# henry123-boy/Level-S2FM_official

Hardware: AMD Instinct MI355X
Metric: rendered rays/sec (fwd+bwd) (higher is better)
Workload: dtype f32; 1 GPU; C2: ETH3D bounds, 1024 rays x 128 samples per GPU, dual field, L16/F2/T19 hash grid, fwd+loss+bwd; rays_per_gpu=1024, samples_per_ray=128, dual_field=True, parallelism=dp1 (rays sharded by view)

## Files before the change

level-s2fm_official_amd/csrc/bin_items.h:

```cpp
#pragma once

#include "render_common.h"

namespace {

constexpr int kAccSlots = 2 << kSlabShift;
constexpr int kSlabBins = 128 << (13 - kSlabShift);
constexpr int kBins = kSlabBins;
#ifndef LS2FM_FILL_TILE
#define LS2FM_FILL_TILE 256
#endif
constexpr int kCountThreads = LS2FM_FILL_TILE;
constexpr int kFillThreads = LS2FM_FILL_TILE;
constexpr int kFillCap = kFillThreads * 17 / 4;
#ifndef LS2FM_FILL_WIN
#define LS2FM_FILL_WIN (LS2FM_FILL_TILE * 17 / 8)
#endif
constexpr int kFillWin = LS2FM_FILL_WIN;
#ifndef LS2FM_ACC_THREADS
#define LS2FM_ACC_THREADS 1024
#endif
constexpr int kAccThreads = LS2FM_ACC_THREADS;
#ifndef LS2FM_ACC_BATCH
#define LS2FM_ACC_BATCH 4
// ... 184 lines not shown

inline int* scan_ticket(const BinMeta& bm) { return reinterpret_cast<int*>(bm.level_bound) + 48; }
__device__ __forceinline__ int* scan_ticket_dev(const BinMeta& bm) { return reinterpret_cast<int*>(bm.level_bound) + 48; }
__host__ __device__ __forceinline__ int* acc_claim(const BinMeta& bm) { return reinterpret_cast<int*>(bm.level_bound) + 50; }

__device__ __forceinline__ int wave_scan_incl_i32(int v, int lane) {
#pragma unroll
    for (int o = 1; o < 64; o <<= 1) {
        const int t = __shfl_up(v, o, 64);
        if (lane >= o) v += t;
    }
    return v;
}

constexpr int kScanTiles = 512;
constexpr int kScanArenaInts = kScanTiles * kScanGroup + (512 / kScanGroup) * kScanGroup + LS2FM_MAX_LEVELS + 1;
[[maybe_unused]] __device__ void scan_job_run(const ScanJob& sj, const int job, const int tid, const int nt, int* arena) {
    int* stage = arena;
    int (*chunk_sum)[kScanGroup] = reinterpret_cast<int (*)[kScanGroup]>(arena + kScanTiles * kScanGroup);
    int* level_total = arena + kScanTiles * kScanGroup + (512 / kScanGroup) * kScanGroup;
    int& s_last = level_total[LS2FM_MAX_LEVELS];
    const BinMeta& bm = sj.bm;
    const int l = job / kScanJobsPerLevel;
    const int sub = tid % kScanGroup, ch = tid / kScanGroup, n_ch = nt / kScanGroup;
    const int b0 = (job % kScanJobsPerLevel) * kScanGroup;
    int* blk = bm.tile + (int64_t)l * bm.n_tiles * kBins + b0;
    int carry = 0;
    for (int base = 0; base < bm.n_tiles; base += kScanTiles) {
        const int nt_here = bm.n_tiles - base < kScanTiles ? bm.n_tiles - base : kScanTiles;
        for (int e = tid; e < nt_here * kScanGroup; e += nt)
            stage[e] = blk[(int64_t)(base + e / kScanGroup) * kBins + e % kScanGroup];
        __syncthreads();
        const int per = (nt_here + n_ch - 1) / n_ch;
        const int t0 = ch * per, t1 = t0 + per < nt_here ? t0 + per : nt_here;
        int sum = 0;
        for (int t = t0; t < t1; ++t) sum += stage[t * kScanGroup + sub];
        chunk_sum[ch][sub] = sum;
        __syncthreads();
        int run = carry, total = carry;
        for (int q = 0; q < n_ch; ++q) {
            const int v = chunk_sum[q][sub];
            if (q < ch) run += v;
            total += v;
        }
// ... 4 lines not shown
        }
        carry = total;
        __syncthreads();
        for (int e = tid; e < nt_here * kScanGroup; e += nt)
            blk[(int64_t)(base + e / kScanGroup) * kBins + e % kScanGroup] = stage[e];
        __syncthreads();
    }
    if (ch == 0) __hip_atomic_store(&bm.count[l * kBins + b0 + sub], carry, __ATOMIC_RELAXED, __HIP_MEMORY_SCOPE_AGENT);
    asm volatile("s_waitcnt vmcnt(0)" ::: "memory");
    __syncthreads();
    if (tid == 0) s_last = atomicAdd(scan_ticket_dev(bm), 1) == sj.n_levels * kScanJobsPerLevel - 1;
    __syncthreads();
    if (!s_last) return;
    const int lane = tid & 63, wave = tid >> 6, n_waves = nt >> 6;
    constexpr int kChunks = (kBins + 63) / 64;
    constexpr int kHeld = 4;
    int held[kHeld][kChunks];
#pragma unroll
    for (int h = 0; h < kHeld; ++h) {
        const int lv = wave + h * n_waves;
        int tot = 0;
#pragma unroll
        for (int c = 0; c < kChunks; ++c) {
            const int bb = 64 * c + lane;
            held[h][c] = (lv < sj.n_levels && bb < kBins)
                             ? __hip_atomic_load(&bm.count[lv * kBins + bb], __ATOMIC_RELAXED, __HIP_MEMORY_SCOPE_AGENT) : 0;
            tot += held[h][c];
        }
#pragma unroll
        for (int o = 32; o > 0; o >>= 1) tot += __shfl_xor(tot, o, 64);
        if (lane == 0 && lv < LS2FM_MAX_LEVELS) level_total[lv] = tot;
    }
    __syncthreads();
#pragma unroll
    for (int h = 0; h < kHeld; ++h) {
        const int lv = wave + h * n_waves;
        if (lv >= sj.n_levels) continue;
        int before = 0;
        for (int q = 0; q < lv; ++q) before += level_total[q];
        int run2 = 0;
#pragma unroll
        for (int c = 0; c < kChunks; ++c) {
            const int bb = 64 * c + lane;
            const int cnt = held[h][c];
            const int incl = wave_scan_incl_i32(cnt, lane);
            if (bb < kBins) bm.start[lv * kBins + bb] = before + run2 + incl - cnt;
            run2 += __shfl(incl, 63, 64);
        }
    }
    if (tid == 0) *scan_ticket_dev(bm) = 0;
}

struct ZeroJob { float4* a; int64_t na; float4* b; int64_t nb; float4* c; int64_t nc; int blocks; };
__device__ __forceinline__ void zero_job_run(const ZeroJob& z, const int job, const int tid, const int nt) {
    const float4 zero = make_float4(0.f, 0.f, 0.f, 0.f);
    const int64_t stride = (int64_t)z.blocks * nt;
    for (int64_t i = (int64_t)job * nt + tid; i < z.na; i += stride) z.a[i] = zero;
    for (int64_t i = (int64_t)job * nt + tid; i < z.nb; i += stride) z.b[i] = zero;
    for (int64_t i = (int64_t)job * nt + tid; i < z.nc; i += stride) z.c[i] = zero;
// ... 4 lines not shown
```

level-s2fm_official_amd/csrc/loss_head.hip:

```cpp
#include "bin_items.h"

namespace {

constexpr int kLossThreads = 256;
constexpr int kLossMaxBlocks = 512;
constexpr int kSums = 8;

struct LossIn {
    const float* rgb; const float* rgb_gt;
    const float* normals;
    const float* depth; const float* depth_ref;
    const uint8_t* mask_eik; const uint8_t* mask_dc; const uint8_t* mask_mse;
    int64_t n_rays; int32_t n_samples;
};

__device__ __forceinline__ float smooth_l1(float d) { const float a = fabsf(d); return a < 1.0f ? 0.5f * d * d : a - 0.5f; }
__device__ __forceinline__ float smooth_l1_grad(float d) { return fabsf(d) < 1.0f ? d : (d > 0.f ? 1.0f : -1.0f); }
__device__ __forceinline__ float sign_of(float d) { return d > 0.f ? 1.0f : (d < 0.f ? -1.0f : 0.f); }

__device__ __forceinline__ void finish_terms(const double* s, const float* w, float* terms, double* sums_out) {
    const float rgb = (float)(s[0] / s[1]);
    const float eik = (float)(s[2] / s[3]);
    const float dc = s[5] > 0.0 ? (float)(s[4] / s[5]) : 0.f;
    const float mse = (float)(s[6] / s[7]);
    terms[0] = rgb; terms[1] = eik; terms[2] = dc; terms[3] = mse;
    terms[4] = fmaf(w[2], dc, fmaf(w[1], eik, w[0] * rgb));
    terms[5] = terms[4];
    terms[6] = -10.0f * log10f(mse);
    terms[7] = 0.f;
    for (int k = 0; k < kSums; ++k) sums_out[k] = s[k];
}

__global__ void __launch_bounds__(kLossThreads)
loss_head_fwd_kernel(LossIn in, const float* __restrict__ weights, double* __restrict__ partial, unsigned* __restrict__ ticket,
                     double* __restrict__ sums_out, float* __restrict__ terms) {
    __shared__ double red[kLossThreads / 64][kSums];
    __shared__ bool last;
    const int tid = threadIdx.x, lane = tid & 63, wave = tid >> 6;
    const int64_t n_points = in.n_rays * in.n_samples;
    const int64_t stride = (int64_t)gridDim.x * kLossThreads;
    double s[kSums];
#pragma unroll
    for (int k = 0; k < kSums; ++k) s[k] = 0.0;
    for (int64_t i = (int64_t)blockIdx.x * kLossThreads + tid; i < n_points; i += stride) {
        const int64_t r = i / in.n_samples;
        if (in.mask_eik && !in.mask_eik[r]) continue;
// ... 83 lines not shown
            const float d = in.rgb[3 * i + c] - in.rgb_gt[3 * i + c];
            float v = g_rgb * sign_of(d);
            if (m) v = fmaf(g_mse * 2.0f, d, v);
            d_rgb[3 * i + c] = v;
        }
        float gd = 0.f;
        if (in.depth_ref && (!in.mask_dc || in.mask_dc[i])) gd = g_dc * smooth_l1_grad(in.depth_ref[i] - in.depth[i]);
        d_depth[i] = -gd;
        if (d_depth_ref) d_depth_ref[i] = gd;
    }
}

constexpr int kPostThreads = 512;
__global__ void __launch_bounds__(kPostThreads)
post_shade_kernel(ls2fm_loss_spec loss, const float* __restrict__ lpart, int64_t n_rays, int64_t r_pad, int n_samples, ScanJob scan) {
    __shared__ int arena[kScanArenaInts];
    const int tid = threadIdx.x, lane = tid & 63, wave = tid >> 6;
    if (blockIdx.x > 0) {
        scan_job_run(scan, (int)blockIdx.x - 1, tid, kPostThreads, arena);
        return;
    }
    if (loss.rgb_gt == nullptr) return;
    double (*red)[kSums] = reinterpret_cast<double (*)[kSums]>(arena);
    static_assert(sizeof(double) * (kPostThreads / 64) * kSums <= sizeof(int) * kScanArenaInts, "reduction buffer fits");
    double s[kSums];
#pragma unroll
    for (int k = 0; k < kSums; ++k) s[k] = 0.0;
    for (int64_t r = tid; r < n_rays; r += kPostThreads) {
        s[0] += (double)lpart[0 * r_pad + r];
        s[1] += 3.0;
        if (ls2fm_in_eik(loss, r)) { s[2] += (double)lpart[1 * r_pad + r]; s[3] += (double)n_samples; }
        if (loss.depth_ref != nullptr && (loss.mask_dc == nullptr || loss.mask_dc[r])) {
            s[4] += (double)ls2fm_smooth_l1(loss.depth_ref[r] - lpart[2 * r_pad + r]);
            s[5] += 1.0;
        }
        if (ls2fm_in_mse(loss, r)) { s[6] += (double)lpart[3 * r_pad + r]; s[7] += 3.0; }
    }
#pragma unroll
    for (int k = 0; k < kSums; ++k) {
        double v = s[k];
#pragma unroll
        for (int o = 32; o > 0; o >>= 1) v += __shfl_xor(v, o, 64);
        if (lane == 0) red[wave][k] = v;
    }
    __syncthreads();
    if (tid < kSums) {
        double v = 0.0;
        for (int q = 0; q < kPostThreads / 64; ++q) v += red[q][tid];
        if ((tid & 1) && loss.count_scale > 1u) v *= (double)loss.count_scale;
        red[0][tid] = v;
    }
    __syncthreads();
    if (tid == 0) finish_terms(red[0], loss.weights, loss.terms, loss.sums);
}

__global__ void terms_from_sums_kernel(const double* __restrict__ sums, const float* __restrict__ weights, float* __restrict__ terms) {
    double s[kSums], keep[kSums];
    for (int k = 0; k < kSums; ++k) s[k] = sums[k];
    finish_terms(s, weights, terms, keep);
}

}

int ls2fm_launch_post_shade(const ls2fm_loss_spec* loss, const float* ray_part, int64_t n_rays, int n_samples,
                            const ls2fm_grid_desc* scan_grid, int64_t n_points, float* bins_ws, hipStream_t stream) {
    if (!loss && !scan_grid) return LS2FM_OK;
    ls2fm_loss_spec ls{};
    if (loss) ls = *loss;
// ... 64 lines not shown
```

level-s2fm_official_amd/csrc/render_common.h:

```cpp
#pragma once

#include "ls2fm_device.h"

enum ls2fm_prof_id {
    LS2FM_PROF_PREP = 0, LS2FM_PROF_ENCODE_SDF, LS2FM_PROF_ENCODE_RAD, LS2FM_PROF_SHADE_FWD, LS2FM_PROF_SHADE_BWD,
    LS2FM_PROF_WGRAD_GEO, LS2FM_PROF_WGRAD_TAIL, LS2FM_PROF_SCATTER_SDF, LS2FM_PROF_SCATTER_RAD, LS2FM_PROF_FINALIZE,
    LS2FM_PROF_SDF_EVAL, LS2FM_PROF_SPHERE_TRACE, LS2FM_PROF_BIN, LS2FM_PROF_LOSS_FWD,
    LS2FM_PROF_LOSS_BWD, LS2FM_PROF_WGRAD_MLP, LS2FM_PROF_POSE, LS2FM_PROF_ENCODE_PAIR, LS2FM_PROF_COUNT
};
bool ls2fm_prof_enabled();
void ls2fm_prof_begin(int id, hipStream_t stream);
void ls2fm_prof_end(int id, hipStream_t stream);

struct SideCtx { hipStream_t side; hipEvent_t fork, mid, join; };
bool ls2fm_side_stream(SideCtx* out, hipStream_t caller);
int ls2fm_join_on_error(bool forked, const SideCtx& sc, hipStream_t caller, int status);
int* ls2fm_async_error_word(hipStream_t stream);
int ls2fm_device_cus();

constexpr int kHidden = LS2FM_HIDDEN;
constexpr int kOut = LS2FM_FEAT + 1;
constexpr int kInMax = 3 + 2 * LS2FM_MAX_LEVELS;
constexpr int kView = LS2FM_VIEW_ENC;
constexpr int kRadIn = 3 + 3 + kView + 2 * LS2FM_FEAT;
// ... 147 lines not shown
    return (q & 1) ? cosf(x) : sinf(x);
}

static inline bool same_grid_geometry(const ls2fm_grid_desc* a, const ls2fm_grid_desc* b) {
    if (a->n_levels != b->n_levels) return false;
    for (int l = 0; l < a->n_levels; ++l)
        if (a->scale[l] != b->scale[l] || a->resolution[l] != b->resolution[l] || a->size[l] != b->size[l] ||
            a->hashed[l] != b->hashed[l])
            return false;
    return true;
}

int64_t ls2fm_bins_workspace_floats(int n_levels, int64_t n_points);
int ls2fm_explicit_levels(const ls2fm_grid_desc* grid, int dual, int n_samples);

struct WsLayout {
    int64_t p, p_pad, r_pad;
    int l1, l2, dual;
    int64_t packed, e1, j1, e2, sdfv, nrm, rgbs, fe, fe2, rout, lpart;
    int64_t rec1, rec2, rpt, bins, v, p3, gf, dz, gf2, dzr, renc, dexyz, dlen, mpart, wg, dbeta, smax;
    int64_t total;
};

#ifndef LS2FM_SLAB_SHIFT
#define LS2FM_SLAB_SHIFT 13
#endif
constexpr int kSlabShift = LS2FM_SLAB_SHIFT;
static inline int ls2fm_slab_shift(int dual) { return dual ? kSlabShift - 1 : kSlabShift; }
constexpr int kWgradMlpBlocks = 256;
constexpr int kRegsSdf = 48 + 16 + 16 + 5;
constexpr int kRegsGeo = 48 + 16 + 4;
constexpr int kRegsDec = 20;
constexpr int kL1Seg = 16;
struct WgPartLayout {
// ... 45 lines not shown
    w.l1 = l1; w.l2 = l2; w.dual = dual;
    int64_t o = 0;
    auto take = [&](int64_t n) { const int64_t at = o; o += (n + 63) / 64 * 64; return at; };
    const int64_t P = w.p_pad;
    w.packed = take((sizeof(Packed) + 3) / 4);
    w.e1 = take(2 * l1 * P);
    w.j1 = take(6 * l1 * P);
    w.e2 = take(dual ? 2 * l2 * P : 0);
    w.sdfv = take(P);
    w.nrm = take(3 * P);
    w.rgbs = take(3 * P);
    w.fe = take(16 * P);
    w.fe2 = take(dual ? 16 * P : 0);
    w.rout = take(4 * w.r_pad);
    w.lpart = take(4 * w.r_pad);
    w.rpt = take(8 * P);
    w.rec1 = take(4 * (int64_t)l1 * P);
    w.rec2 = take(dual ? 2 * (int64_t)l2 * P : 0);
    w.v = take(35 * P);
    w.p3 = take(3 * P);
    w.gf = take(17 * P);
    w.dz = take(3 * P);
    w.gf2 = take(dual ? 17 * P : 0);
    w.dexyz = take(6 * P);
    w.dlen = take(w.r_pad);
    w.dzr = take(3 * w.r_pad);
    w.renc = take(27 * w.r_pad);
    w.mpart = take(make_wg_part_layout(dual, n_rays, n_samples).total);
    w.wg = take(kWgBlockFloats);
    w.dbeta = take(2 * w.r_pad);
// ... 52 lines not shown

struct Ls2fmWgradParts { const float* sdf; const float* geo; const float* dec; int nb_sdf, nb_geo, nb_dec, dual; };
struct Ls2fmWgradExtra { WsLayout w; const float* ws; void* ready; };
int ls2fm_launch_wgrad_mlp(const FieldC& fc, int dual, int ch1, int ch2, const WsLayout& w, const Packed* pk, const float* center,
                           const float* ray, int64_t n_rays, float* ws, hipStream_t s, bool sdf_only = false,
                           Ls2fmWgradParts* defer = nullptr, const Ls2fmWgradExtra* extra = nullptr, int fused_wgrad = 0);

int ls2fm_points_bwd_front(const ls2fm_field_desc* field, const ls2fm_grid_desc* grid, const ls2fm_params* params, const float* p,
                           int64_t n, const float* d_sdf, const float* d_feat, const float* d_normal, float* zero_table, bool want_dp,
                           void* workspace, hipStream_t s, WsLayout* w_out, hipEvent_t rows_ready);
int ls2fm_points_bwd_scatter(const ls2fm_field_desc* field, const ls2fm_grid_desc* grid, int64_t n, void* workspace, float* table,
                             int add_into, hipStream_t s, int phase);

int ls2fm_launch_shade_fwd(const FieldC& fc, int dual, int ch1, int ch2, const Packed* pk, const float* center, const float* ray,
                           int64_t n_rays, const WsLayout& w, float* ws, float* rgb, float* sdfs_volume, float* normals,
                           float* depth_mlp, float* normal_mlp, const ls2fm_loss_spec* loss, hipStream_t s);
```

level-s2fm_official_amd/csrc/render_fwd.hip:

```cpp
#include <cmath>

#include "bin_items.h"

namespace {

struct LayerRef { const float* v; const float* g; const float* b; int out, in; };

__device__ __forceinline__ LayerRef layer_ref(const ls2fm_params& P, int li, int in_dim, int rad_in) {
    switch (li) {
        case 0: return {P.sdf_mlp[0].weight_v, P.sdf_mlp[0].weight_g, P.sdf_mlp[0].bias, kHidden, in_dim};
        case 1: return {P.sdf_mlp[1].weight_v, P.sdf_mlp[1].weight_g, P.sdf_mlp[1].bias, kOut, kHidden};
        case 2: return {P.geo_mlp[0].weight_v, P.geo_mlp[0].weight_g, P.geo_mlp[0].bias, kHidden, in_dim};
        case 3: return {P.geo_mlp[1].weight_v, P.geo_mlp[1].weight_g, P.geo_mlp[1].bias, kOut, kHidden};
        case 4: return {P.rad_mlp[0].weight_v, P.rad_mlp[0].weight_g, P.rad_mlp[0].bias, kHidden, rad_in};
        case 5: return {P.rad_mlp[1].weight_v, P.rad_mlp[1].weight_g, P.rad_mlp[1].bias, kHidden, kHidden};
        default: return {P.rad_mlp[2].weight_v, P.rad_mlp[2].weight_g, P.rad_mlp[2].bias, 3, kHidden};
    }
}

__device__ __forceinline__ int row_base(int li) {
    switch (li) {
        case 0: return 0;
        case 1: return 64;
        case 2: return 81;
// ... 195 lines not shown
    prep_weights_task(P, in_dim, in_dim2, rad_in, dual, with_rad, out, (int)blockIdx.x, (int)threadIdx.x, kPrepThreads);
}

struct XcdPlan { int start[9]; };

#ifdef LS2FM_STAMPS
__device__ unsigned long long g_enc_ticks[2 * LS2FM_MAX_LEVELS + 24];
#endif

struct EncodeExtras {
    ls2fm_params params;
    int in_dim, in_dim2, rad_in, dual;
    Packed* packed;
    int* tile_counts;
    int* scan_ticket;
    int n_tiles, sshift;
    int n_explicit;
    int n_prep_tasks;
    const float* pts;
};

constexpr int kEncThreads = 512;
constexpr int kEncRows = kEncThreads / kFillTile;
static_assert(kEncThreads % kFillTile == 0, "a gather workgroup covers whole tiles");
constexpr int kEncReserved = 8;

struct LevelOne { float scale; uint32_t res, size, offset, hashed; };

__device__ __forceinline__ void locate_sample(const FieldC& fc, const float* __restrict__ center, const float* __restrict__ ray,
                                              const float* __restrict__ pts, int64_t i, const LevelOne& lv, uint32_t g[3], Cell& c) {
// ... 21 lines not shown
#ifndef LS2FM_ENC_MINW
#define LS2FM_ENC_MINW 1
#endif
template <bool INTERLEAVED>
__global__ void __launch_bounds__(kEncThreads, LS2FM_ENC_MINW)
ray_encode_kernel(LevelSet lv1, LevelSet lv2, FieldC fc, const float* __restrict__ center, const float* __restrict__ ray,
                  const float* __restrict__ table1, const float* __restrict__ table2, int64_t n_points, int64_t p_pad,
                  int n_chunks, XcdPlan plan, float* __restrict__ enc1, float* __restrict__ enc2, float* __restrict__ jac,
                  EncodeExtras ex) {
    __shared__ int hist[kEncRows][kBins];
    const int tid = threadIdx.x;
    if (blockIdx.x < kEncReserved) {
        if (ex.packed && (int)blockIdx.x < ex.n_prep_tasks)
            prep_weights_task(ex.params, ex.in_dim, ex.in_dim2, ex.rad_in, ex.dual, 1, ex.packed, (int)blockIdx.x, tid, kEncThreads);
        if (blockIdx.x == 3 && tid == 0 && ex.scan_ticket) *ex.scan_ticket = 0;
        return;
    }
    const int bx = (int)blockIdx.x - kEncReserved;
    const int xcd = bx & 7, j = bx >> 3;
    const int unit = plan.start[xcd] + j;
    if (unit >= plan.start[xcd + 1]) return;
    const int pl = unit / n_chunks;
    const int chunk = unit % n_chunks;
    const bool two = !INTERLEAVED && table2 != nullptr;
    const bool second = two && (pl & 1);
    const int l = two ? pl >> 1 : pl;
    LevelOne lv;
    lv.scale = second ? lv2.scale[l] : lv1.scale[l];
    lv.res = second ? lv2.res[l] : lv1.res[l];
    lv.size = second ? lv2.size[l] : lv1.size[l];
// ... 210 lines not shown

int ls2fm_launch_points_encode(const ls2fm_field_desc* field, const ls2fm_grid_desc* grid, const ls2fm_params* params,
                               const float* pts, const WsLayout& w, float* ws, hipStream_t s) {
    const FieldC fc = make_field_c(field);
    const int L = grid->n_levels;
    const int n_chunks = (int)((w.p + kEncThreads - 1) / kEncThreads);
    int most = 0;
    const XcdPlan plan = make_xcd_plan(grid, L, nullptr, 0, 1, n_chunks, true, &most);
    EncodeExtras ex;
    ex.params = *params;
    ex.in_dim = 3 + 2 * L; ex.in_dim2 = 0; ex.rad_in = 0; ex.dual = 0;
    ex.packed = (Packed*)(ws + w.packed);
    const BinMeta bm = make_bin_meta(ws + w.bins, w.p);
    ex.tile_counts = bm.tile;
    ex.scan_ticket = scan_ticket(bm);
    ex.n_tiles = bm.n_tiles;
    ex.sshift = ls2fm_slab_shift(0);
    ex.n_explicit = 0;
    ex.n_prep_tasks = 1;
    ex.pts = pts;
    ray_encode_kernel<false><<<(unsigned)(kEncReserved + 8 * most), kEncThreads, 0, s>>>(
        make_level_set(grid), make_level_set(grid), fc, nullptr, nullptr, params->sdf_table, nullptr, w.p, w.p_pad, n_chunks, plan,
        ws + w.e1, nullptr, ws + w.j1, ex);
    return ls2fm_launch_status();
}
int ls2fm_launch_image_encode(const ls2fm_field_desc* field, const ls2fm_grid_desc* sdf_grid, const ls2fm_grid_desc* rad_grid,
                              const ls2fm_params* params, const float* center, const float* ray, int64_t n_points, int64_t p_pad,
                              float* e1, float* e2, float* j1, Packed* packed, hipStream_t s) {
    const FieldC fc = make_field_c(field);
    const int dual = field->dual_field ? 1 : 0;
    const int L1 = sdf_grid->n_levels, L2 = dual ? rad_grid->n_levels : 0;
    const int n_chunks = (int)((n_points + kEncThreads - 1) / kEncThreads);
    const bool interleaved = dual && params->dual_table;
    const bool pair = dual && !interleaved;
    int most = 0;
    const XcdPlan plan = make_xcd_plan(sdf_grid, L1, pair ? rad_grid : nullptr, pair ? L2 : 0, field->n_samples, n_chunks, false, &most,
                                       interleaved);
    EncodeExtras ex;
    ex.params = *params;
    ex.in_dim = 3 + 2 * L1; ex.in_dim2 = 3 + 2 * L2; ex.rad_in = 3 + 3 + kView + LS2FM_FEAT * (dual ? 2 : 1); ex.dual = dual;
    ex.packed = packed;
    ex.tile_counts = nullptr; ex.scan_ticket = nullptr; ex.n_tiles = 0; ex.sshift = ls2fm_slab_shift(dual);
    ex.n_explicit = 0;
    ex.n_prep_tasks = 3; ex.pts = nullptr;
    const unsigned enc_blocks = (unsigned)(kEncReserved + 8 * most);
    const int enc_span = dual ? LS2FM_PROF_ENCODE_PAIR : LS2FM_PROF_ENCODE_SDF;
    ls2fm_prof_begin(enc_span, s);
    if (interleaved)
        ray_encode_kernel<true><<<enc_blocks, kEncThreads, 0, s>>>(
            make_level_set(sdf_grid), make_level_set(sdf_grid), fc, center, ray, params->dual_table, nullptr, n_points, p_pad, n_chunks,
            plan, e1, e2, j1, ex);
    else
        ray_encode_kernel<false><<<enc_blocks, kEncThreads, 0, s>>>(
            make_level_set(sdf_grid), make_level_set(pair ? rad_grid : sdf_grid), fc, center, ray, params->sdf_table,
            pair ? params->rad_table : nullptr, n_points, p_pad, n_chunks, plan, e1, pair ? e2 : nullptr, j1, ex);
    ls2fm_prof_end(enc_span, s);
    return ls2fm_launch_status();
// ... 28 lines not shown

    const int n_chunks = (int)((w.p + kEncThreads - 1) / kEncThreads);
    const bool interleaved = dual && params->dual_table;
    const bool pair = dual && !interleaved;
    const int enc_span = dual ? LS2FM_PROF_ENCODE_PAIR : LS2FM_PROF_ENCODE_SDF;
    int most = 0;
    const XcdPlan plan = make_xcd_plan(sdf_grid, L1, pair ? rad_grid : nullptr, pair ? L2 : 0, field->n_samples, n_chunks, prepare_bwd, &most,
                                       interleaved);
    EncodeExtras ex;
    ex.params = *params;
    ex.in_dim = 3 + 2 * L1; ex.in_dim2 = 3 + 2 * L2; ex.rad_in = 3 + 3 + kView + LS2FM_FEAT * (dual ? 2 : 1); ex.dual = dual;
    ex.packed = pk;
    ex.tile_counts = nullptr; ex.scan_ticket = nullptr; ex.n_tiles = 0; ex.sshift = ls2fm_slab_shift(dual);
    ex.n_explicit = ls2fm_explicit_levels(sdf_grid, dual, field->n_samples);
    ex.n_prep_tasks = 3; ex.pts = nullptr;
    if (prepare_bwd) {
        const BinMeta bm = make_bin_meta(ws + w.bins, w.p);
        ex.tile_counts = bm.tile;
        ex.scan_ticket = scan_ticket(bm);
        ex.n_tiles = bm.n_tiles;
    }
    const unsigned enc_blocks = (unsigned)(kEncReserved + 8 * most);
    ls2fm_prof_begin(enc_span, s);
    if (interleaved)
        ray_encode_kernel<true><<<enc_blocks, kEncThreads, 0, s>>>(
            make_level_set(sdf_grid), make_level_set(sdf_grid), fc, center, ray, params->dual_table, nullptr, w.p, w.p_pad, n_chunks,
            plan, ws + w.e1, ws + w.e2, ws + w.j1, ex);
    else
        ray_encode_kernel<false><<<enc_blocks, kEncThreads, 0, s>>>(
            make_level_set(sdf_grid), make_level_set(pair ? rad_grid : sdf_grid), fc, center, ray, params->sdf_table,
            pair ? params->rad_table : nullptr, w.p, w.p_pad, n_chunks, plan, ws + w.e1, pair ? ws + w.e2 : nullptr, ws + w.j1, ex);
    ls2fm_prof_end(enc_span, s);

    ls2fm_prof_begin(LS2FM_PROF_SHADE_FWD, s);
    ls2fm_launch_shade_fwd(fc, dual, 2 * L1, 2 * L2, pk, center, ray, n_rays, w, ws, rgb, sdfs_volume, normals, depth_mlp,
                           normal_mlp, loss, s);
    ls2fm_prof_end(LS2FM_PROF_SHADE_FWD, s);
    if (loss && opts->loss_inputs_ready && hipStreamWaitEvent(s, (hipEvent_t)opts->loss_inputs_ready, 0) != hipSuccess)
        return LS2FM_ERR_LAUNCH;
    ls2fm_prof_begin(LS2FM_PROF_BIN, s);
    const int st = ls2fm_launch_post_shade(loss, ws + w.lpart, n_rays, field->n_samples, prepare_bwd ? sdf_grid : nullptr, w.p,
                                           ws + w.bins, s);
    ls2fm_prof_end(LS2FM_PROF_BIN, s);
    if (st != LS2FM_OK) return st;
    return ls2fm_launch_status();
}
```

level-s2fm_official_amd/csrc/render_image.hip:

```cpp
#include "camera_ray.h"
#include "shade_fwd.h"

#ifndef LS2FM_IMAGE_CHUNK_MB
#define LS2FM_IMAGE_CHUNK_MB 640
#endif

namespace {

constexpr int kRayThreads = 256;

__global__ void __launch_bounds__(kRayThreads)
image_rays_kernel(const float* __restrict__ poses, Kinv K, int64_t hw, int width, int64_t g0, int64_t n, float* __restrict__ centers,
                  float* __restrict__ rays) {
    const int64_t i = (int64_t)blockIdx.x * kRayThreads + threadIdx.x;
    if (i >= n) return;
    const int64_t g = g0 + i;
    const int64_t v = g / hw, p = g - v * hw;
    float pose[12];
#pragma unroll
    for (int q = 0; q < 12; ++q) pose[q] = poses[12 * v + q];
    float c2w[3][4];
    camera_to_world(pose, c2w);
    const float x = (float)(p % width) + 0.5f;
    const float y = (float)(p / width) + 0.5f;
// ... 6 lines not shown
                   const float* __restrict__ ray, int64_t p_pad, const float* __restrict__ E1, const float* __restrict__ J1,
                   const float* __restrict__ E2, float* __restrict__ rgb_out, float* __restrict__ depth_out,
                   float* __restrict__ nm_out, float* __restrict__ op_out) {
    constexpr bool SAVE = false;
    float* const sdfs_out = nullptr;
    float* const normals_out = nullptr;
    float* const SDFV = nullptr;
    float* const NRM = nullptr;
    float* const RGBS = nullptr;
    float* const FE = nullptr;
    float* const FE2 = nullptr;
    float* const ROUT = nullptr;
    float* const LPART = nullptr;
    const int64_t r_pad = 0;
    const ls2fm_loss_spec loss{};
#include "shade_fwd_body.inc"
}

struct ImageLayout {
    int64_t chunk_rays, p_pad;
    int64_t packed, center, ray, e1, j1, e2, total;
};

ImageLayout make_image_layout(const ls2fm_field_desc* field, int l1, int l2) {
    ImageLayout m;
    const int N = field->n_samples;
    const int64_t floats_per_point = 8 * (int64_t)l1 + 2 * (int64_t)l2;
    int64_t points = ((int64_t)LS2FM_IMAGE_CHUNK_MB << 20) / (4 * floats_per_point);
    if (points > LS2FM_MAX_RENDER_POINTS) points = LS2FM_MAX_RENDER_POINTS;
    m.chunk_rays = points / N > 0 ? points / N : 1;
// ... 84 lines not shown
```

level-s2fm_official_amd/csrc/shade_fwd.hip:

```cpp
#include "shade_fwd.h"

namespace {

template <bool DUAL, int MAXS, int CT, bool FULL = false>
__global__ void __launch_bounds__(MAXS * 4 / CT, CT == 2 ? 4 : 2)
shade_fwd_kernel(FieldC fc, int ch1_arg, int ch2_arg, const Packed* __restrict__ pk, const float* __restrict__ center,
                 const float* __restrict__ ray, int64_t p_pad, const float* __restrict__ E1,
                 const float* __restrict__ J1, const float* __restrict__ E2, float* __restrict__ rgb_out,
                 float* __restrict__ sdfs_out, float* __restrict__ normals_out, float* __restrict__ depth_out,
                 float* __restrict__ nm_out, float* __restrict__ SDFV, float* __restrict__ NRM,
                 float* __restrict__ RGBS, float* __restrict__ FE, float* __restrict__ FE2, float* __restrict__ ROUT,
                 float* __restrict__ LPART, int64_t r_pad, ls2fm_loss_spec loss) {
    constexpr bool SAVE = true;
    float* const op_out = nullptr;
#include "shade_fwd_body.inc"
}

}

int ls2fm_launch_shade_fwd(const FieldC& fc, int dual, int ch1, int ch2, const Packed* pk, const float* center, const float* ray,
                           int64_t n_rays, const WsLayout& w, float* ws, float* rgb, float* sdfs_volume, float* normals,
                           float* depth_mlp, float* normal_mlp, const ls2fm_loss_spec* loss, hipStream_t s) {
    const bool small = fc.n_samples <= 256;
    const int per_wave = small ? 32 : 64;
    const int threads = (fc.n_samples + per_wave - 1) / per_wave * 64;
    ls2fm_loss_spec ls{};
    if (loss) ls = *loss;
    const bool full = small && ch1 == 32 && (!dual || ch2 == 32) && fc.n_samples % 32 == 0;
#define LS2FM_SHADE_FWD(DUAL, MAXS, CT, FULL)                                                                      \
    shade_fwd_kernel<DUAL, MAXS, CT, FULL><<<(unsigned)n_rays, threads, 0, s>>>(                                    \
        fc, ch1, ch2, pk, center, ray, w.p_pad, ws + w.e1, ws + w.j1, DUAL ? ws + w.e2 : nullptr, rgb, sdfs_volume, \
        normals, depth_mlp, normal_mlp, ws + w.sdfv, ws + w.nrm, ws + w.rgbs, ws + w.fe, DUAL ? ws + w.fe2 : nullptr,        \
        ws + w.rout, ws + w.lpart, w.r_pad, ls)
    if (dual) { if (full) LS2FM_SHADE_FWD(true, 256, 2, true); else if (small) LS2FM_SHADE_FWD(true, 256, 2, false); else LS2FM_SHADE_FWD(true, 512, 4, false); }
    else      { if (full) LS2FM_SHADE_FWD(false, 256, 2, true); else if (small) LS2FM_SHADE_FWD(false, 256, 2, false); else LS2FM_SHADE_FWD(false, 512, 4, false); }
#undef LS2FM_SHADE_FWD
    return LS2FM_OK;
}
```

level-s2fm_official_amd/csrc/shade_fwd_body.inc:

```
    __shared__ float s_part[MAXS / (16 * CT)][10];
    __shared__ float s_view[3];
    __shared__ float s_x[MAXS][8];
    __shared__ float s_w[kMfmaSdfFloats];
    const int N = fc.n_samples;
    const int ch1 = FULL ? 32 : ch1_arg, ch2 = FULL ? 32 : ch2_arg;
    const int64_t r = blockIdx.x;
    const int n = threadIdx.x, lane = n & 63, wave = n >> 6, n_waves = blockDim.x >> 6;
    const int jl = lane & 15, g = lane >> 4;
    const RayGeom gm = load_ray(fc, center, ray, r);
    const MfmaW& mw = pk->mw;
    {
        const float4* src = reinterpret_cast<const float4*>(&mw.sdf);
        float4* dst = reinterpret_cast<float4*>(s_w);
        for (int q = n; q < kMfmaSdfFloats / 4; q += blockDim.x) dst[q] = src[q];
    }
    const float* __restrict__ s_w0a = s_w;
    const float* __restrict__ s_w1a = s_w + 4 * 9 * 64;
    const float* __restrict__ s_w0ta = s_w + kMfmaFieldFloats;
    const float* __restrict__ s_w10 = s_w0ta + 3 * 4 * 4 * 64;

    if (wave == 0) {
        const float e = lane < kView ? view_component(gm.d, lane) : 0.f;
#pragma unroll
        for (int c = 0; c < 3; ++c) {
// ... 333 lines not shown
#pragma unroll
        for (int a = 0; a < 3; ++a) nm_out[r * 3 + a] = tot[4 + a] + rest * nrm_n[a];
        if (!SAVE && op_out != nullptr) op_out[r] = tot[7];
        if (SAVE && loss.rgb_gt != nullptr) {
            float l1 = 0.f, sq = 0.f;
#pragma unroll
            for (int c = 0; c < 3; ++c) {
                const float d = rgb_r[c] - loss.rgb_gt[r * 3 + c];
                l1 += fabsf(d);
                sq = fmaf(d, d, sq);
                ROUT[c * r_pad + r] = rgb_r[c];
            }
            ROUT[3 * r_pad + r] = depth_r;
            float eik = 0.f;
            for (int w = 0; w < n_waves; ++w) eik += s_part[w][9];
            LPART[0 * r_pad + r] = l1;
            LPART[1 * r_pad + r] = eik;
            LPART[2 * r_pad + r] = depth_r;
            LPART[3 * r_pad + r] = ls2fm_in_mse(loss, r) ? sq : 0.f;
        }
    }
```

Before: 2.540 million rays/s.

## Fuse bin scan and loss reduction into shade forward tail via tickets

Removes the separate post-shade kernel by having each shade_fwd block grab a ticket at its end. Blocks use that ticket to run scan jobs through the shared s_w arena, and the last block to finish runs the loss reduction. The loss reduction moves into a shared header with a fixed virtual-thread count, and the scan's final pass now reloads counts instead of holding them in registers. The intent is to save one kernel launch and its serialization point. The cost is extra atomics, an extra sync at the end of every shade block, and reliance on correct cross-block memory ordering.

Measured after the change: 2.532 million rays/s. No clear change (-0.3%).

```diff
diff --git a/level-s2fm_official_amd/csrc/bin_items.h b/level-s2fm_official_amd/csrc/bin_items.h
--- a/level-s2fm_official_amd/csrc/bin_items.h
+++ b/level-s2fm_official_amd/csrc/bin_items.h
@@ -222,11 +222,13 @@
 }
 
 constexpr int kScanTiles = 512;
-constexpr int kScanArenaInts = kScanTiles * kScanGroup + (512 / kScanGroup) * kScanGroup + LS2FM_MAX_LEVELS + 1;
-[[maybe_unused]] __device__ void scan_job_run(const ScanJob& sj, const int job, const int tid, const int nt, int* arena) {
+constexpr int scan_arena_ints(int tiles, int max_nt) { return tiles * kScanGroup + (max_nt / kScanGroup) * kScanGroup + LS2FM_MAX_LEVELS + 1; }
+constexpr int kScanArenaInts = scan_arena_ints(kScanTiles, 512);
+template <int TILES = kScanTiles, int MAXNT = 512>
+[[maybe_unused]] __device__ __forceinline__ void scan_job_run(const ScanJob& sj, const int job, const int tid, const int nt, int* arena) {
     int* stage = arena;
-    int (*chunk_sum)[kScanGroup] = reinterpret_cast<int (*)[kScanGroup]>(arena + kScanTiles * kScanGroup);
-    int* level_total = arena + kScanTiles * kScanGroup + (512 / kScanGroup) * kScanGroup;
+    int (*chunk_sum)[kScanGroup] = reinterpret_cast<int (*)[kScanGroup]>(arena + TILES * kScanGroup);
+    int* level_total = arena + TILES * kScanGroup + (MAXNT / kScanGroup) * kScanGroup;
     int& s_last = level_total[LS2FM_MAX_LEVELS];
     const BinMeta& bm = sj.bm;
     const int l = job / kScanJobsPerLevel;
@@ -234,8 +236,8 @@
     const int b0 = (job % kScanJobsPerLevel) * kScanGroup;
     int* blk = bm.tile + (int64_t)l * bm.n_tiles * kBins + b0;
     int carry = 0;
-    for (int base = 0; base < bm.n_tiles; base += kScanTiles) {
-        const int nt_here = bm.n_tiles - base < kScanTiles ? bm.n_tiles - base : kScanTiles;
+    for (int base = 0; base < bm.n_tiles; base += TILES) {
+        const int nt_here = bm.n_tiles - base < TILES ? bm.n_tiles - base : TILES;
         for (int e = tid; e < nt_here * kScanGroup; e += nt)
             stage[e] = blk[(int64_t)(base + e / kScanGroup) * kBins + e % kScanGroup];
         __syncthreads();
@@ -270,35 +272,26 @@
     if (!s_last) return;
     const int lane = tid & 63, wave = tid >> 6, n_waves = nt >> 6;
     constexpr int kChunks = (kBins + 63) / 64;
-    constexpr int kHeld = 4;
-    int held[kHeld][kChunks];
-#pragma unroll
-    for (int h = 0; h < kHeld; ++h) {
-        const int lv = wave + h * n_waves;
+    for (int lv = wave; lv < sj.n_levels; lv += n_waves) {
         int tot = 0;
 #pragma unroll
         for (int c = 0; c < kChunks; ++c) {
             const int bb = 64 * c + lane;
-            held[h][c] = (lv < sj.n_levels && bb < kBins)
-                             ? __hip_atomic_load(&bm.count[lv * kBins + bb], __ATOMIC_RELAXED, __HIP_MEMORY_SCOPE_AGENT) : 0;
-            tot += held[h][c];
+            tot += bb < kBins ? __hip_atomic_load(&bm.count[lv * kBins + bb], __ATOMIC_RELAXED, __HIP_MEMORY_SCOPE_AGENT) : 0;
         }
 #pragma unroll
         for (int o = 32; o > 0; o >>= 1) tot += __shfl_xor(tot, o, 64);
-        if (lane == 0 && lv < LS2FM_MAX_LEVELS) level_total[lv] = tot;
+        if (lane == 0) level_total[lv] = tot;
     }
     __syncthreads();
-#pragma unroll
-    for (int h = 0; h < kHeld; ++h) {
-        const int lv = wave + h * n_waves;
-        if (lv >= sj.n_levels) continue;
+    for (int lv = wave; lv < sj.n_levels; lv += n_waves) {
         int before = 0;
         for (int q = 0; q < lv; ++q) before += level_total[q];
         int run2 = 0;
 #pragma unroll
         for (int c = 0; c < kChunks; ++c) {
             const int bb = 64 * c + lane;
-            const int cnt = held[h][c];
+            const int cnt = bb < kBins ? __hip_atomic_load(&bm.count[lv * kBins + bb], __ATOMIC_RELAXED, __HIP_MEMORY_SCOPE_AGENT) : 0;
             const int incl = wave_scan_incl_i32(cnt, lane);
             if (bb < kBins) bm.start[lv * kBins + bb] = before + run2 + incl - cnt;
             run2 += __shfl(incl, 63, 64);
diff --git a/level-s2fm_official_amd/csrc/loss_head.hip b/level-s2fm_official_amd/csrc/loss_head.hip
--- a/level-s2fm_official_amd/csrc/loss_head.hip
+++ b/level-s2fm_official_amd/csrc/loss_head.hip
@@ -1,10 +1,10 @@
 #include "bin_items.h"
+#include "loss_reduce.h"
 
 namespace {
 
 constexpr int kLossThreads = 256;
 constexpr int kLossMaxBlocks = 512;
-constexpr int kSums = 8;
 
 struct LossIn {
     const float* rgb; const float* rgb_gt;
@@ -17,19 +17,6 @@
 __device__ __forceinline__ float smooth_l1(float d) { const float a = fabsf(d); return a < 1.0f ? 0.5f * d * d : a - 0.5f; }
 __device__ __forceinline__ float smooth_l1_grad(float d) { return fabsf(d) < 1.0f ? d : (d > 0.f ? 1.0f : -1.0f); }
 __device__ __forceinline__ float sign_of(float d) { return d > 0.f ? 1.0f : (d < 0.f ? -1.0f : 0.f); }
-
-__device__ __forceinline__ void finish_terms(const double* s, const float* w, float* terms, double* sums_out) {
-    const float rgb = (float)(s[0] / s[1]);
-    const float eik = (float)(s[2] / s[3]);
-    const float dc = s[5] > 0.0 ? (float)(s[4] / s[5]) : 0.f;
-    const float mse = (float)(s[6] / s[7]);
-    terms[0] = rgb; terms[1] = eik; terms[2] = dc; terms[3] = mse;
-    terms[4] = fmaf(w[2], dc, fmaf(w[1], eik, w[0] * rgb));
-    terms[5] = terms[4];
-    terms[6] = -10.0f * log10f(mse);
-    terms[7] = 0.f;
-    for (int k = 0; k < kSums; ++k) sums_out[k] = s[k];
-}
 
 __global__ void __launch_bounds__(kLossThreads)
 loss_head_fwd_kernel(LossIn in, const float* __restrict__ weights, double* __restrict__ partial, unsigned* __restrict__ ticket,
@@ -143,44 +130,15 @@
 constexpr int kPostThreads = 512;
 __global__ void __launch_bounds__(kPostThreads)
 post_shade_kernel(ls2fm_loss_spec loss, const float* __restrict__ lpart, int64_t n_rays, int64_t r_pad, int n_samples, ScanJob scan) {
-    __shared__ int arena[kScanArenaInts];
-    const int tid = threadIdx.x, lane = tid & 63, wave = tid >> 6;
+    __shared__ __attribute__((aligned(16))) int arena[kScanArenaInts];
+    const int tid = threadIdx.x;
     if (blockIdx.x > 0) {
         scan_job_run(scan, (int)blockIdx.x - 1, tid, kPostThreads, arena);
         return;
     }
     if (loss.rgb_gt == nullptr) return;
-    double (*red)[kSums] = reinterpret_cast<double (*)[kSums]>(arena);
-    static_assert(sizeof(double) * (kPostThreads / 64) * kSums <= sizeof(int) * kScanArenaInts, "reduction buffer fits");
-    double s[kSums];
-#pragma unroll
-    for (int k = 0; k < kSums; ++k) s[k] = 0.0;
-    for (int64_t r = tid; r < n_rays; r += kPostThreads) {
-        s[0] += (double)lpart[0 * r_pad + r];
-        s[1] += 3.0;
-        if (ls2fm_in_eik(loss, r)) { s[2] += (double)lpart[1 * r_pad + r]; s[3] += (double)n_samples; }
-        if (loss.depth_ref != nullptr && (loss.mask_dc == nullptr || loss.mask_dc[r])) {
-            s[4] += (double)ls2fm_smooth_l1(loss.depth_ref[r] - lpart[2 * r_pad + r]);
-            s[5] += 1.0;
-        }
-        if (ls2fm_in_mse(loss, r)) { s[6] += (double)lpart[3 * r_pad + r]; s[7] += 3.0; }
-    }
-#pragma unroll
-    for (int k = 0; k < kSums; ++k) {
-        double v = s[k];
-#pragma unroll
-        for (int o = 32; o > 0; o >>= 1) v += __shfl_xor(v, o, 64);
-        if (lane == 0) red[wave][k] = v;
-    }
-    __syncthreads();
-    if (tid < kSums) {
-        double v = 0.0;
-        for (int q = 0; q < kPostThreads / 64; ++q) v += red[q][tid];
-        if ((tid & 1) && loss.count_scale > 1u) v *= (double)loss.count_scale;
-        red[0][tid] = v;
-    }
-    __syncthreads();
-    if (tid == 0) finish_terms(red[0], loss.weights, loss.terms, loss.sums);
+    static_assert(sizeof(double) * (kLossVirtual / 64) * kSums <= sizeof(int) * kScanArenaInts, "reduction buffer fits");
+    loss_reduce_rows<false>(loss, lpart, n_rays, r_pad, n_samples, tid, kPostThreads, reinterpret_cast<double (*)[kSums]>(arena));
 }
 
 __global__ void terms_from_sums_kernel(const double* __restrict__ sums, const float* __restrict__ weights, float* __restrict__ terms) {
diff --git a/level-s2fm_official_amd/csrc/loss_reduce.h b/level-s2fm_official_amd/csrc/loss_reduce.h
--- /dev/null
+++ b/level-s2fm_official_amd/csrc/loss_reduce.h
@@ -0,0 +1,63 @@
+#pragma once
+
+#include "wgrad_tail.h"
+
+namespace {
+
+constexpr int kSums = 8;
+constexpr int kLossVirtual = 512;
+
+__device__ __forceinline__ void finish_terms(const double* s, const float* w, float* terms, double* sums_out) {
+    const float rgb = (float)(s[0] / s[1]);
+    const float eik = (float)(s[2] / s[3]);
+    const float dc = s[5] > 0.0 ? (float)(s[4] / s[5]) : 0.f;
+    const float mse = (float)(s[6] / s[7]);
+    terms[0] = rgb; terms[1] = eik; terms[2] = dc; terms[3] = mse;
+    terms[4] = fmaf(w[2], dc, fmaf(w[1], eik, w[0] * rgb));
+    terms[5] = terms[4];
+    terms[6] = -10.0f * log10f(mse);
+    terms[7] = 0.f;
+    for (int k = 0; k < kSums; ++k) sums_out[k] = s[k];
+}
+
+template <bool WT>
+__device__ __forceinline__ void loss_reduce_rows(const ls2fm_loss_spec& loss, const float* __restrict__ lpart, int64_t n_rays,
+                                                 int64_t r_pad, int n_samples, const int tid, const int nt, double (*red)[kSums]) {
+    const int lane = tid & 63;
+    for (int vt = tid; vt < kLossVirtual; vt += nt) {
+        double s[kSums];
+#pragma unroll
+        for (int k = 0; k < kSums; ++k) s[k] = 0.0;
+        for (int64_t r = vt; r < n_rays; r += kLossVirtual) {
+            float p0, p1, p2, p3;
+            if (WT) wg_load4(lpart + r, lpart + r_pad + r, lpart + 2 * r_pad + r, lpart + 3 * r_pad + r, p0, p1, p2, p3);
+            else { p0 = lpart[r]; p1 = lpart[r_pad + r]; p2 = lpart[2 * r_pad + r]; p3 = lpart[3 * r_pad + r]; }
+            s[0] += (double)p0;
+            s[1] += 3.0;
+            if (ls2fm_in_eik(loss, r)) { s[2] += (double)p1; s[3] += (double)n_samples; }
+            if (loss.depth_ref != nullptr && (loss.mask_dc == nullptr || loss.mask_dc[r])) {
+                s[4] += (double)ls2fm_smooth_l1(loss.depth_ref[r] - p2);
+                s[5] += 1.0;
+            }
+            if (ls2fm_in_mse(loss, r)) { s[6] += (double)p3; s[7] += 3.0; }
+        }
+#pragma unroll
+        for (int k = 0; k < kSums; ++k) {
+            double v = s[k];
+#pragma unroll
+            for (int o = 32; o > 0; o >>= 1) v += __shfl_xor(v, o, 64);
+            if (lane == 0) red[vt >> 6][k] = v;
+        }
+    }
+    __syncthreads();
+    if (tid < kSums) {
+        double v = 0.0;
+        for (int q = 0; q < kLossVirtual / 64; ++q) v += red[q][tid];
+        if ((tid & 1) && loss.count_scale > 1u) v *= (double)loss.count_scale;
+        red[0][tid] = v;
+    }
+    __syncthreads();
+    if (tid == 0) finish_terms(red[0], loss.weights, loss.terms, loss.sums);
+}
+
+}
diff --git a/level-s2fm_official_amd/csrc/render_common.h b/level-s2fm_official_amd/csrc/render_common.h
--- a/level-s2fm_official_amd/csrc/render_common.h
+++ b/level-s2fm_official_amd/csrc/render_common.h
@@ -185,10 +185,13 @@
 int64_t ls2fm_bins_workspace_floats(int n_levels, int64_t n_points);
 int ls2fm_explicit_levels(const ls2fm_grid_desc* grid, int dual, int n_samples);
 
+constexpr int kFwdTicketGroups = 64;
+constexpr int kFwdTicketInts = 128;
+
 struct WsLayout {
     int64_t p, p_pad, r_pad;
     int l1, l2, dual;
-    int64_t packed, e1, j1, e2, sdfv, nrm, rgbs, fe, fe2, rout, lpart;
+    int64_t packed, e1, j1, e2, sdfv, nrm, rgbs, fe, fe2, rout, lpart, ltick;
     int64_t rec1, rec2, rpt, bins, v, p3, gf, dz, gf2, dzr, renc, dexyz, dlen, mpart, wg, dbeta, smax;
     int64_t total;
 };
@@ -264,6 +267,7 @@
     w.fe2 = take(dual ? 16 * P : 0);
     w.rout = take(4 * w.r_pad);
     w.lpart = take(4 * w.r_pad);
+    w.ltick = take(kFwdTicketInts);
     w.rpt = take(8 * P);
     w.rec1 = take(4 * (int64_t)l1 * P);
     w.rec2 = take(dual ? 2 * (int64_t)l2 * P : 0);
@@ -346,4 +350,5 @@
 
 int ls2fm_launch_shade_fwd(const FieldC& fc, int dual, int ch1, int ch2, const Packed* pk, const float* center, const float* ray,
                            int64_t n_rays, const WsLayout& w, float* ws, float* rgb, float* sdfs_volume, float* normals,
-                           float* depth_mlp, float* normal_mlp, const ls2fm_loss_spec* loss, hipStream_t s);
+                           float* depth_mlp, float* normal_mlp, const ls2fm_loss_spec* loss, bool finish_inside,
+                           const ls2fm_grid_desc* scan_grid, hipStream_t s);
diff --git a/level-s2fm_official_amd/csrc/render_fwd.hip b/level-s2fm_official_amd/csrc/render_fwd.hip
--- a/level-s2fm_official_amd/csrc/render_fwd.hip
+++ b/level-s2fm_official_amd/csrc/render_fwd.hip
@@ -233,6 +233,7 @@
     Packed* packed;
     int* tile_counts;
     int* scan_ticket;
+    int* fwd_ticket;
     int n_tiles, sshift;
     int n_explicit;
     int n_prep_tasks;
@@ -284,6 +285,7 @@
         if (ex.packed && (int)blockIdx.x < ex.n_prep_tasks)
             prep_weights_task(ex.params, ex.in_dim, ex.in_dim2, ex.rad_in, ex.dual, 1, ex.packed, (int)blockIdx.x, tid, kEncThreads);
         if (blockIdx.x == 3 && tid == 0 && ex.scan_ticket) *ex.scan_ticket = 0;
+        if (blockIdx.x == 3 && tid <= kFwdTicketGroups && ex.fwd_ticket) ex.fwd_ticket[tid] = 0;
         return;
     }
     const int bx = (int)blockIdx.x - kEncReserved;
@@ -524,6 +526,7 @@
     const BinMeta bm = make_bin_meta(ws + w.bins, w.p);
     ex.tile_counts = bm.tile;
     ex.scan_ticket = scan_ticket(bm);
+    ex.fwd_ticket = nullptr;
     ex.n_tiles = bm.n_tiles;
     ex.sshift = ls2fm_slab_shift(0);
     ex.n_explicit = 0;
@@ -550,7 +553,7 @@
     ex.params = *params;
     ex.in_dim = 3 + 2 * L1; ex.in_dim2 = 3 + 2 * L2; ex.rad_in = 3 + 3 + kView + LS2FM_FEAT * (dual ? 2 : 1); ex.dual = dual;
     ex.packed = packed;
-    ex.tile_counts = nullptr; ex.scan_ticket = nullptr; ex.n_tiles = 0; ex.sshift = ls2fm_slab_shift(dual);
+    ex.tile_counts = nullptr; ex.scan_ticket = nullptr; ex.fwd_ticket = nullptr; ex.n_tiles = 0; ex.sshift = ls2fm_slab_shift(dual);
     ex.n_explicit = 0;
     ex.n_prep_tasks = 3; ex.pts = nullptr;
     const unsigned enc_blocks = (unsigned)(kEncReserved + 8 * most);
@@ -609,6 +612,8 @@
     ex.tile_counts = nullptr; ex.scan_ticket = nullptr; ex.n_tiles = 0; ex.sshift = ls2fm_slab_shift(dual);
     ex.n_explicit = ls2fm_explicit_levels(sdf_grid, dual, field->n_samples);
     ex.n_prep_tasks = 3; ex.pts = nullptr;
+    const bool finish_inside = (loss || prepare_bwd) && !(loss && opts->loss_inputs_ready);
+    ex.fwd_ticket = finish_inside ? reinterpret_cast<int*>(ws + w.ltick) : nullptr;
     if (prepare_bwd) {
         const BinMeta bm = make_bin_meta(ws + w.bins, w.p);
         ex.tile_counts = bm.tile;
@@ -629,8 +634,9 @@
 
     ls2fm_prof_begin(LS2FM_PROF_SHADE_FWD, s);
     ls2fm_launch_shade_fwd(fc, dual, 2 * L1, 2 * L2, pk, center, ray, n_rays, w, ws, rgb, sdfs_volume, normals, depth_mlp,
-                           normal_mlp, loss, s);
+                           normal_mlp, loss, finish_inside, prepare_bwd ? sdf_grid : nullptr, s);
     ls2fm_prof_end(LS2FM_PROF_SHADE_FWD, s);
+    if (finish_inside) return ls2fm_launch_status();
     if (loss && opts->loss_inputs_ready && hipStreamWaitEvent(s, (hipEvent_t)opts->loss_inputs_ready, 0) != hipSuccess)
         return LS2FM_ERR_LAUNCH;
     ls2fm_prof_begin(LS2FM_PROF_BIN, s);
diff --git a/level-s2fm_official_amd/csrc/render_image.hip b/level-s2fm_official_amd/csrc/render_image.hip
--- a/level-s2fm_official_amd/csrc/render_image.hip
+++ b/level-s2fm_official_amd/csrc/render_image.hip
@@ -1,5 +1,7 @@
 #include "camera_ray.h"
 #include "shade_fwd.h"
+#include "bin_items.h"
+#include "loss_reduce.h"
 
 #ifndef LS2FM_IMAGE_CHUNK_MB
 #define LS2FM_IMAGE_CHUNK_MB 640
@@ -44,6 +46,10 @@
     float* const LPART = nullptr;
     const int64_t r_pad = 0;
     const ls2fm_loss_spec loss{};
+    int* const LTICK = nullptr;
+    const int64_t n_rays_all = 0;
+    int* const SCAN_META = nullptr;
+    const int scan_tiles = 0, scan_levels = 0;
 #include "shade_fwd_body.inc"
 }
 
diff --git a/level-s2fm_official_amd/csrc/shade_fwd.hip b/level-s2fm_official_amd/csrc/shade_fwd.hip
--- a/level-s2fm_official_amd/csrc/shade_fwd.hip
+++ b/level-s2fm_official_amd/csrc/shade_fwd.hip
@@ -1,4 +1,6 @@
 #include "shade_fwd.h"
+#include "bin_items.h"
+#include "loss_reduce.h"
 
 namespace {
 
@@ -10,7 +12,8 @@
                  float* __restrict__ sdfs_out, float* __restrict__ normals_out, float* __restrict__ depth_out,
                  float* __restrict__ nm_out, float* __restrict__ SDFV, float* __restrict__ NRM,
                  float* __restrict__ RGBS, float* __restrict__ FE, float* __restrict__ FE2, float* __restrict__ ROUT,
-                 float* __restrict__ LPART, int64_t r_pad, ls2fm_loss_spec loss) {
+                 float* __restrict__ LPART, int64_t r_pad, ls2fm_loss_spec loss, int* __restrict__ LTICK,
+                 int64_t n_rays_all, int* __restrict__ SCAN_META, int scan_tiles, int scan_levels) {
     constexpr bool SAVE = true;
     float* const op_out = nullptr;
 #include "shade_fwd_body.inc"
@@ -20,18 +23,27 @@
 
 int ls2fm_launch_shade_fwd(const FieldC& fc, int dual, int ch1, int ch2, const Packed* pk, const float* center, const float* ray,
                            int64_t n_rays, const WsLayout& w, float* ws, float* rgb, float* sdfs_volume, float* normals,
-                           float* depth_mlp, float* normal_mlp, const ls2fm_loss_spec* loss, hipStream_t s) {
+                           float* depth_mlp, float* normal_mlp, const ls2fm_loss_spec* loss, bool finish_inside,
+                           const ls2fm_grid_desc* scan_grid, hipStream_t s) {
     const bool small = fc.n_samples <= 256;
     const int per_wave = small ? 32 : 64;
     const int threads = (fc.n_samples + per_wave - 1) / per_wave * 64;
     ls2fm_loss_spec ls{};
     if (loss) ls = *loss;
+    int* ltick = finish_inside ? reinterpret_cast<int*>(ws + w.ltick) : nullptr;
+    int* scan_meta = nullptr;
+    int scan_tiles = 0, scan_levels = 0;
+    if (finish_inside && scan_grid) {
+        scan_meta = reinterpret_cast<int*>(ws + w.bins);
+        scan_tiles = make_bin_meta(ws + w.bins, w.p).n_tiles;
+        scan_levels = scan_grid->n_levels;
+    }
     const bool full = small && ch1 == 32 && (!dual || ch2 == 32) && fc.n_samples % 32 == 0;
 #define LS2FM_SHADE_FWD(DUAL, MAXS, CT, FULL)                                                                      \
     shade_fwd_kernel<DUAL, MAXS, CT, FULL><<<(unsigned)n_rays, threads, 0, s>>>(                                    \
         fc, ch1, ch2, pk, center, ray, w.p_pad, ws + w.e1, ws + w.j1, DUAL ? ws + w.e2 : nullptr, rgb, sdfs_volume, \
         normals, depth_mlp, normal_mlp, ws + w.sdfv, ws + w.nrm, ws + w.rgbs, ws + w.fe, DUAL ? ws + w.fe2 : nullptr,        \
-        ws + w.rout, ws + w.lpart, w.r_pad, ls)
+        ws + w.rout, ws + w.lpart, w.r_pad, ls, ltick, n_rays, scan_meta, scan_tiles, scan_levels)
     if (dual) { if (full) LS2FM_SHADE_FWD(true, 256, 2, true); else if (small) LS2FM_SHADE_FWD(true, 256, 2, false); else LS2FM_SHADE_FWD(true, 512, 4, false); }
     else      { if (full) LS2FM_SHADE_FWD(false, 256, 2, true); else if (small) LS2FM_SHADE_FWD(false, 256, 2, false); else LS2FM_SHADE_FWD(false, 512, 4, false); }
 #undef LS2FM_SHADE_FWD
diff --git a/level-s2fm_official_amd/csrc/shade_fwd_body.inc b/level-s2fm_official_amd/csrc/shade_fwd_body.inc
--- a/level-s2fm_official_amd/csrc/shade_fwd_body.inc
+++ b/level-s2fm_official_amd/csrc/shade_fwd_body.inc
@@ -1,7 +1,7 @@
     __shared__ float s_part[MAXS / (16 * CT)][10];
     __shared__ float s_view[3];
     __shared__ float s_x[MAXS][8];
-    __shared__ float s_w[kMfmaSdfFloats];
+    __shared__ __attribute__((aligned(16))) float s_w[kMfmaSdfFloats];
     const int N = fc.n_samples;
     const int ch1 = FULL ? 32 : ch1_arg, ch2 = FULL ? 32 : ch2_arg;
     const int64_t r = blockIdx.x;
@@ -371,9 +371,43 @@
             ROUT[3 * r_pad + r] = depth_r;
             float eik = 0.f;
             for (int w = 0; w < n_waves; ++w) eik += s_part[w][9];
-            LPART[0 * r_pad + r] = l1;
-            LPART[1 * r_pad + r] = eik;
-            LPART[2 * r_pad + r] = depth_r;
-            LPART[3 * r_pad + r] = ls2fm_in_mse(loss, r) ? sq : 0.f;
-        }
-    }
+            wg_store(&LPART[0 * r_pad + r], l1);
+            wg_store(&LPART[1 * r_pad + r], eik);
+            wg_store(&LPART[2 * r_pad + r], depth_r);
+            wg_store(&LPART[3 * r_pad + r], ls2fm_in_mse(loss, r) ? sq : 0.f);
+        }
+    }
+
+    if (SAVE && LTICK != nullptr) {
+        __shared__ int s_ticket[2];
+        if (n == N - 1) {
+            asm volatile("s_waitcnt vmcnt(0)" ::: "memory");
+            const int classes = n_rays_all < kFwdTicketGroups ? (int)n_rays_all : kFwdTicketGroups;
+            const int cls = (int)(r % kFwdTicketGroups);
+            const int members = (int)((n_rays_all - cls + kFwdTicketGroups - 1) / kFwdTicketGroups);
+            const int t = atomicAdd(&LTICK[1 + cls], 1);
+            int last = 0;
+            if (t == members - 1) last = atomicAdd(&LTICK[0], 1) == classes - 1;
+            s_ticket[0] = t * classes + cls;
+            s_ticket[1] = last;
+        }
+        __syncthreads();
+        if (SCAN_META != nullptr) {
+            ScanJob scan;
+            scan.bm.count = SCAN_META;
+            scan.bm.start = SCAN_META + LS2FM_MAX_LEVELS * kBins;
+            scan.bm.level_bound = reinterpret_cast<float*>(SCAN_META + 2 * LS2FM_MAX_LEVELS * kBins);
+            scan.bm.tile = SCAN_META + 3 * LS2FM_MAX_LEVELS * kBins + 64;
+            scan.bm.n_tiles = scan_tiles;
+            scan.n_levels = scan_levels;
+            constexpr int kTiles = (kMfmaSdfFloats - (1024 / kScanGroup) * kScanGroup - LS2FM_MAX_LEVELS - 1) / kScanGroup / 64 * 64;
+            static_assert(scan_arena_ints(kTiles, 1024) <= kMfmaSdfFloats && kTiles >= 64, "the scan's staging area fits s_w");
+            const int n_jobs = scan.n_levels * kScanJobsPerLevel;
+            for (int64_t job = s_ticket[0]; job < n_jobs; job += n_rays_all)
+                scan_job_run<kTiles, 1024>(scan, (int)job, n, (int)blockDim.x, reinterpret_cast<int*>(s_w));
+        }
+        if (s_ticket[1] && loss.rgb_gt != nullptr) {
+            __syncthreads();
+            loss_reduce_rows<true>(loss, LPART, n_rays_all, r_pad, N, n, (int)blockDim.x, reinterpret_cast<double (*)[kSums]>(s_w));
+        }
+    }
```
